# dmeoli/optiml

Measured on AMD Instinct MI355X. Metric: dual_qp_iterations_per_sec, higher is better.
Workload: dtype f64

## Files before the change

### optiml_amd/csrc/bq_api.hip

```cpp
#include <algorithm>
#include <chrono>
#include <cmath>
#include <cstdarg>
#include <cstdlib>

#include "bq_al.h"
#include "bq_c7.h"

static thread_local std::string g_last_error;

void bq_set_error(const char *fmt, ...) {
    char buf[1024];
    va_list ap;
    va_start(ap, fmt);
    vsnprintf(buf, sizeof(buf), fmt, ap);
    va_end(ap);
    g_last_error = buf;
}

extern "C" const char *bq_last_error(void) { return g_last_error.c_str(); }
extern "C" int bq_abi_version(void) { return BQ_ABI_VERSION; }

extern "C" int bq_device_count(int *count) {
    BQ_ARG(count != nullptr, "count is NULL");
// ... 692 lines not shown

extern "C" int bq_problem_eval(bq_problem *p, const double *x, double *f, double *g) {
    BQ_ARG(p && x && f, "NULL argument");
    BQ_HIP(hipSetDevice(p->ctx->device));
    BQ_TRY(upload_padded(p, x, p->va, p->N, p->ldN));
    BQ_TRY(bq_problem_apply(p, p->va, p->vb, nullptr));
    BQ_TRY(bq_vec_eval_f(p, p->va, p->vb, g ? p->vb : nullptr, p->scal));
    BQ_HIP(hipMemcpyAsync(f, p->scal, sizeof(double), hipMemcpyDeviceToHost, p->ctx->stream));
    if (g) BQ_HIP(hipMemcpyAsync(g, p->vb, sizeof(double) * p->N, hipMemcpyDeviceToHost, p->ctx->stream));
    BQ_SYNC(p->ctx);
    return BQ_OK;
}

extern "C" int bq_problem_gram_matvec(bq_problem *p, const double *w, double *out) {
    BQ_ARG(p && w && out, "NULL argument");
    BQ_ARG(p->kernel >= 0, "not a kernel-structured problem");
    bq_ctx *c = p->ctx;
    BQ_HIP(hipSetDevice(c->device));
    BQ_HIP(hipMemsetAsync(p->w, 0, sizeof(double) * p->ld, c->stream));
    BQ_HIP(hipMemcpyAsync(p->w, w, sizeof(double) * p->n, hipMemcpyHostToDevice, c->stream));
    BQ_TRY(bq_panel_product(p, false, p->w, nullptr));
    BQ_HIP(hipMemcpyAsync(out, p->s, sizeof(double) * p->n, hipMemcpyDeviceToHost, c->stream));
    BQ_SYNC(c);
    return BQ_OK;
}

extern "C" int bq_problem_panel_rows(bq_problem *p, int64_t row0, int64_t nrows, double *out) {
    BQ_ARG(p && out, "NULL argument");
    BQ_ARG(row0 >= p->r0 && row0 + nrows <= p->r1 && nrows >= 0, "rows outside this rank's block");
    BQ_ARG(!p->streamed, "a streamed problem keeps no panel");
    bq_ctx *c = p->ctx;
    BQ_HIP(hipSetDevice(c->device));
    if (nrows == 0) return BQ_OK;
    if (p->symmetric && p->compact) {
        const bq_c7p pv = bq_c7_view(p->panel, p->panel_elems);
        std::vector<uint32_t> lo((size_t)p->n);
        std::vector<uint16_t> mid((size_t)p->n);
        std::vector<uint8_t> top((size_t)p->n);
        for (int64_t r = 0; r < nrows; ++r) {
            const int64_t i = row0 + r;
            const int64_t len = std::min(p->n, bq_sym_pitch(i / BQ_SYM_TILE)), a = bq_sym_addr(i, 0, p->I0);
            BQ_HIP(hipMemcpyAsync(lo.data(), pv.lo + a, (size_t)len * 4, hipMemcpyDeviceToHost, c->stream));
            BQ_HIP(hipMemcpyAsync(mid.data(), pv.mid + a, (size_t)len * 2, hipMemcpyDeviceToHost, c->stream));
            BQ_HIP(hipMemcpyAsync(top.data(), pv.top + a, (size_t)len, hipMemcpyDeviceToHost, c->stream));
            BQ_SYNC(c);
            double *o = out + r * p->n;
            for (int64_t j = 0; j < len; ++j) {
                const uint64_t b = bq_c7_bits(lo[j], mid[j], top[j]);
                std::memcpy(&o[j], &b, sizeof(double));
            }
            for (int64_t j = len; j < p->n; ++j) o[j] = 0.0;
        }
        return BQ_OK;
    }
    if (p->symmetric) {
        const size_t esz = p->storage == BQ_F64 ? 8 : 4;
        std::vector<unsigned char> tmp((size_t)p->n * esz);
        for (int64_t r = 0; r < nrows; ++r) {
            const int64_t i = row0 + r;
            const int64_t len = std::min(p->n, bq_sym_pitch(i / BQ_SYM_TILE));
            BQ_HIP(hipMemcpyAsync(tmp.data(), (const unsigned char *)p->panel + (size_t)bq_sym_addr(i, 0, p->I0) * esz,
                                  (size_t)len * esz, hipMemcpyDeviceToHost, c->stream));
            BQ_SYNC(c);
            double *o = out + r * p->n;
            for (int64_t j = 0; j < len; ++j)
                o[j] = p->storage == BQ_F64 ? ((const double *)tmp.data())[j] : (double)((const float *)tmp.data())[j];
            for (int64_t j = len; j < p->n; ++j) o[j] = 0.0;
        }
        return BQ_OK;
    }
    const int64_t lr = row0 - p->r0;
    if (p->storage == BQ_F64) {
        BQ_HIP(hipMemcpy2DAsync(out, p->n * 8, (const double *)p->panel + lr * p->ld, p->ld * 8, p->n * 8, nrows,
                                hipMemcpyDeviceToHost, c->stream));
        BQ_SYNC(c);
    } else {
        std::vector<float> tmp((size_t)nrows * p->n);
        BQ_HIP(hipMemcpy2DAsync(tmp.data(), p->n * 4, (const float *)p->panel + lr * p->ld, p->ld * 4, p->n * 4, nrows,
                                hipMemcpyDeviceToHost, c->stream));
        BQ_SYNC(c);
        for (size_t i = 0; i < tmp.size(); ++i) out[i] = (double)tmp[i];
    }
    return BQ_OK;
}

extern "C" int bq_problem_time_matvec(bq_problem *p, int reps, double *mean_ms) {
    BQ_ARG(p && mean_ms && reps > 0, "argument");
    bq_ctx *c = p->ctx;
    BQ_HIP(hipSetDevice(c->device));
    hipEvent_t e0, e1;
    BQ_HIP(hipEventCreate(&e0));
    BQ_HIP(hipEventCreate(&e1));
    const bool prof = c->profiling;
    c->profiling = false;
    bq_seg_table tab;
    if (p->symmetric) bq_sym_seg_table(p, &tab);
    auto local = [&]() {
        if (p->streamed)
            return bq_stream_sym_product(c, p->stream_img, p->n, p->nb, tab, p->kernel, p->gamma, p->coef0, p->degree, p->add_one, p->w,
                                         p->s, 0, nullptr);
// ... 782 lines not shown
```

### optiml_amd/csrc/bq_common.h

```cpp
#pragma once
#include <hip/hip_runtime.h>

#include <atomic>
#include <cstdint>
#include <cstdio>
#include <cstring>
#include <string>
#include <vector>

#include "../../include/bcqp.h"

void bq_set_error(const char *fmt, ...);

#define BQ_HIP(expr)                                                                          \
    do {                                                                                      \
        hipError_t _e = (expr);                                                               \
        if (_e != hipSuccess) {                                                               \
            bq_set_error("%s failed at %s:%d: %s", #expr, __FILE__, __LINE__, hipGetErrorString(_e)); \
            return BQ_ERR_HIP;                                                                \
        }                                                                                     \
    } while (0)

#define BQ_TRY(expr)              \
    do {                          \
// ... 177 lines not shown
        int have = 0;
        std::vector<double> g, lp, lm;
        std::vector<unsigned char> mL, mU;
    };
    resume_t *resume = nullptr;
};

int bq_prof_begin(bq_ctx *ctx, int which, hipEvent_t *e0, hipEvent_t *e1, bool bracket = true);
int bq_prof_end(bq_ctx *ctx, int which, hipEvent_t e0, hipEvent_t e1, bool recorded = false);
void bq_prof_drop(bq_ctx *ctx, hipEvent_t e0, hipEvent_t e1);
void bq_prof_skip_arg(bq_ctx *ctx, hipEvent_t e0, int **slot, int *seq);
int bq_exchange_rows(bq_ctx *ctx, double *s, int64_t n, int64_t blk, int64_t r0, int64_t r1);
int bq_exchange_sum(bq_ctx *ctx, double *v, int64_t count);
int bq_exchange_gather(bq_ctx *ctx, double *buf, int64_t chunk);
void bq_problem_unref(bq_problem *p);
void bq_ctx_register(bq_ctx *c, bool alive);
void bq_ctx_drop_cache(bq_ctx *ctx);
void *bq_ctx_cache_take(bq_ctx *ctx, size_t bytes, size_t *cap);
void bq_ctx_cache_put(bq_ctx *ctx, void *panel, size_t bytes);
void bq_ctx_hold(bq_ctx *ctx, void *ptr, size_t bytes, const void *owner);
void bq_ctx_release_held(bq_ctx *ctx, const void *owner);

constexpr int BQ_F64C = 16;
struct bq_panel_ref {
    const void *base;
    int storage;
    int64_t elems;
};
static inline bq_panel_ref bq_problem_panel(const bq_problem *p, const void *base = nullptr) {
    return {base ? base : p->panel, p->compact ? BQ_F64C : p->storage, p->panel_elems};
}
static inline bool bq_compact_allowed() { return bq_hook_on("compact_panel"); }

constexpr int64_t BQ_SYM_TILE = 256;
__host__ __device__ inline int64_t bq_sym_off(int64_t I) { return BQ_SYM_TILE * BQ_SYM_TILE * (I * (I + 1) / 2); }
__host__ __device__ inline int64_t bq_sym_pitch(int64_t I) { return (I + 1) * BQ_SYM_TILE; }
__host__ __device__ inline int64_t bq_sym_addr(int64_t i, int64_t j, int64_t I0) {
    const int64_t I = i / BQ_SYM_TILE;
    return bq_sym_off(I) - bq_sym_off(I0) + (i - I * BQ_SYM_TILE) * bq_sym_pitch(I) + j;
}
constexpr int BQ_SYM_SEG = 8;
constexpr int BQ_SYM_SEG_MAX = 64;
static inline int bq_sym_segments(int world) { return BQ_SYM_SEG * ((world + BQ_SYM_SEG - 1) / BQ_SYM_SEG); }
int64_t bq_sym_seg_cut(int64_t nb, int s, int S);
static inline int bq_sym_seg_first(int rank, int world, int S) { return (int)((int64_t)rank * S / world); }
struct bq_seg_table {
    int count;
    int lo, hi;
    int slot[BQ_SYM_SEG_MAX];
    long long cut[BQ_SYM_SEG_MAX + 1];
};
struct bq_epilogue;
int bq_launch_symv(bq_ctx *ctx, const bq_panel_ref &panel, bool add_one, int64_t nb, const bq_seg_table &tab,
                   const double *w, double *slab, double *out, const int *done, const bq_epilogue *epi = nullptr);
int bq_launch_symv_segments(bq_ctx *ctx, const bq_panel_ref &panel, bool add_one, int64_t nb, const bq_seg_table &tab,
                            const double *w, double *slab, double *gath, const int *done);
int bq_launch_symv_segsum(bq_ctx *ctx, int64_t nb, const bq_seg_table &tab, const double *gath, double *out, const int *done,
                          const bq_epilogue *epi = nullptr);
void bq_sym_seg_table(const bq_problem *p, bq_seg_table *tab);
int bq_panel_product(bq_problem *p, bool add_one, const double *w, const int *done, const bq_epilogue *epi = nullptr,
                     bool *fused = nullptr);
constexpr int BQ_SYMM_CK = 4;
int64_t bq_symm_slab_len(int64_t nb);
int bq_launch_symm(bq_problem *p, bool add_one, const double *W, int64_t ldw, int slots, double *slab, double *out,
                   const int *nlive);
constexpr int BQ_SYMMW_CK = 16;
int64_t bq_symmw_slab_len(int64_t nb);
int bq_launch_symmw(bq_problem *p, bool add_one, const double *W, int64_t ldw, int slots, double *slab, double *out,
                    const int *nlive);
struct bq_pairs_plan;
int bq_pairs_plan_create(bq_problem *p, int ncls, const int *cls_tiles, int m, const int *pairs, bq_pairs_plan **out);
void bq_pairs_plan_destroy(bq_pairs_plan *pl);
int64_t bq_pairs_slab_len(const bq_pairs_plan *pl);
// ... 55 lines not shown
```

### optiml_amd/csrc/bq_dense.hip

```cpp
#include <algorithm>

#include "bq_common.h"

namespace {

template <typename T> struct bits_of;
template <> struct bits_of<double> {
    static __device__ __forceinline__ long long get(double v) { return __double_as_longlong(v); }
};
template <> struct bits_of<float> {
    static __device__ __forceinline__ long long get(float v) { return (long long)__float_as_int(v); }
};

template <typename T>
__global__ __launch_bounds__(256) void dense_pack_kernel(const double *__restrict__ tmp, int64_t ldt, int64_t width,
                                                         T *__restrict__ dst, int64_t pitch) {
    const int64_t r = blockIdx.y;
    for (int64_t c = (int64_t)blockIdx.x * 256 + threadIdx.x; c < width; c += (int64_t)gridDim.x * 256)
        dst[r * pitch + c] = (T)tmp[r * ldt + c];
}

template <typename T>
__global__ __launch_bounds__(256) void dense_mirror_diag_kernel(T *__restrict__ diag, int64_t pitch, int rows) {
    const int r = blockIdx.x, c = threadIdx.x;
    if (r < rows && c < rows && c > r) diag[(int64_t)r * pitch + c] = diag[(int64_t)c * pitch + r];
}

template <typename T>
__global__ __launch_bounds__(256) void dense_symcheck_kernel(const double *__restrict__ tmp, int64_t ldt, int64_t c_org, int64_t I,
                                                             int rows, int64_t c_lo, int64_t c_hi, const T *__restrict__ panel,
                                                             int64_t I0, int *__restrict__ flag) {
    __shared__ T tile[32][33];
    const int tx = threadIdx.x & 31, ty = threadIdx.x >> 5;
    const int64_t cb = c_lo + (int64_t)blockIdx.x * 32;
    const int rb = (int)blockIdx.y * 32;
    for (int k = ty; k < 32; k += 8) {
        const int64_t c = cb + k;
        const int r = rb + tx;
        T v = (T)0;
        if (c < c_hi && r < rows) v = panel[bq_sym_addr(c, I * BQ_SYM_TILE + r, I0)];
        tile[k][tx] = v;
    }
    __syncthreads();
    bool bad = false;
    for (int k = ty; k < 32; k += 8) {
        const int r = rb + k;
        const int64_t c = cb + tx;
        if (r < rows && c < c_hi) {
            const T mine = (T)tmp[(int64_t)r * ldt + (c - c_org)];
            bad = bad || bits_of<T>::get(mine) != bits_of<T>::get(tile[tx][k]);
        }
    }
// ... 4 lines not shown
int upload_sym_t(bq_problem *p, const double *Q, bool check, int *symmetric) {
    bq_ctx *c = p->ctx;
    const int64_t n = p->n, T256 = BQ_SYM_TILE;
    *symmetric = 1;
    if (p->I1 <= p->I0) return BQ_OK;
    struct scratch {
        double *tmp = nullptr;
        int *flag = nullptr;
        ~scratch() {
            if (tmp) hipFree(tmp);
            if (flag) hipFree(flag);
        }
    } s;
    const int64_t ldt = p->ld;
    BQ_HIP(hipMalloc(&s.tmp, sizeof(double) * (size_t)T256 * (size_t)ldt));
    BQ_HIP(hipMalloc(&s.flag, sizeof(int)));
    BQ_HIP(hipMemsetAsync(s.flag, 0, sizeof(int), c->stream));
    T *panel = reinterpret_cast<T *>(p->panel);
    const int64_t col_end = std::min(n, p->I1 * T256);
    int seen = 0, blocks = 0;
    auto look = [&]() -> int {
        BQ_HIP(hipMemcpyAsync(&seen, s.flag, sizeof(int), hipMemcpyDeviceToHost, c->stream));
        BQ_SYNC(c);
        return BQ_OK;
    };
    for (int64_t I = p->I1 - 1; I >= p->I0; --I) {
        const int rows = (int)std::min<int64_t>(T256, n - I * T256);
        if (rows <= 0) continue;
        const int64_t lower = std::min(n, (I + 1) * T256);
        const int64_t width = check ? col_end : lower;
        BQ_HIP(hipMemcpy2DAsync(s.tmp, (size_t)ldt * 8, Q + I * T256 * n, (size_t)n * 8, (size_t)width * 8, (size_t)rows,
                                hipMemcpyHostToDevice, c->stream));
        dense_pack_kernel<T><<<dim3((unsigned)std::min<int64_t>((lower + 255) / 256, 1024), (unsigned)rows), 256, 0, c->stream>>>(
            s.tmp, ldt, lower, panel + (bq_sym_off(I) - bq_sym_off(p->I0)), bq_sym_pitch(I));
        if (!check)
            dense_mirror_diag_kernel<T><<<(unsigned)rows, 256, 0, c->stream>>>(panel + (bq_sym_off(I) - bq_sym_off(p->I0)) + I * T256,
                                                                                bq_sym_pitch(I), rows);
        if (check) {
            const int64_t c_lo = I * T256;
            dense_symcheck_kernel<T><<<dim3((unsigned)((col_end - c_lo + 31) / 32), (unsigned)((rows + 31) / 32)), 256, 0, c->stream>>>(
                s.tmp, ldt, 0, I, rows, c_lo, col_end, panel, p->I0, s.flag);
            if (blocks == 0 || blocks % 32 == 31) {
                BQ_TRY(look());
                if (seen) break;
            }
        }
        ++blocks;
        BQ_HIP(hipGetLastError());
    }
    if (check && !seen && p->I0 > 0) {
        const int64_t c_lo = p->I0 * T256;
        for (int64_t Ib = 0; Ib < p->I0; ++Ib) {
            BQ_HIP(hipMemcpy2DAsync(s.tmp, (size_t)ldt * 8, Q + Ib * T256 * n + c_lo, (size_t)n * 8, (size_t)(col_end - c_lo) * 8,
                                    (size_t)T256, hipMemcpyHostToDevice, c->stream));
            dense_symcheck_kernel<T><<<dim3((unsigned)((col_end - c_lo + 31) / 32), (unsigned)(T256 / 32)), 256, 0, c->stream>>>(
                s.tmp, ldt, c_lo, Ib, (int)T256, c_lo, col_end, panel, p->I0, s.flag);
            if (Ib % 32 == 31) {
                BQ_TRY(look());
                if (seen) break;
            }
        }
        BQ_HIP(hipGetLastError());
    }
    if (check) {
        BQ_TRY(look());
        *symmetric = seen ? 0 : 1;
    }
    return BQ_OK;
}

// ... 75 lines not shown
```

### optiml_amd/csrc/bq_gram.hip

```cpp
#include "bq_c7.h"
#include "bq_common.h"

#include "bq_mfma_tile.h"
#include "bq_gram_image.h"

#include <type_traits>
#include <vector>

constexpr int GT = BQ_GT;
#ifndef BQ_STREAM_FOLD
#define BQ_STREAM_FOLD 0
#endif

template <typename T> struct gram_out {
    typedef T *__restrict__ ptr;
    typedef T *row;
};
template <> struct gram_out<bq_c7> {
    typedef bq_c7w ptr;
    typedef bq_c7w row;
};
template <typename T> __device__ __forceinline__ void store_elem(T *p, double v);
template <> __device__ __forceinline__ void store_elem<double>(double *p, double v) { __builtin_nontemporal_store(v, p); }
template <> __device__ __forceinline__ void store_elem<float>(float *p, double v) { __builtin_nontemporal_store((float)v, p); }
__device__ __forceinline__ void store_pair(double *p, double a, double b) {
    bq_d2 v;
    v.x = a;
    v.y = b;
    __builtin_nontemporal_store(v, reinterpret_cast<bq_d2 *>(p));
}
__device__ __forceinline__ void store_pair(float *p, double a, double b) {
    typedef float f2 __attribute__((ext_vector_type(2)));
    f2 v;
    v.x = (float)a;
    v.y = (float)b;
    __builtin_nontemporal_store(v, reinterpret_cast<f2 *>(p));
}

__device__ __forceinline__ void c7_flag(const bq_c7w &p, uint64_t a, uint64_t b) {
    if (!bq_c7_encodable(a) || !bq_c7_encodable(b)) *p.bad = 1;
}
__device__ __forceinline__ void store_pair(const bq_c7w &p, double a, double b) {
// ... 37 lines not shown
__global__ __launch_bounds__(256, 2) void gram_mfma_kernel(gram_params P, typename gram_out<T>::ptr out) {
    __shared__ __attribute__((aligned(16))) bq_tile_smem sm;
    int64_t bx = blockIdx.x, by = blockIdx.y;
    if (P.rect_rb > 0) {
        const int64_t b = blockIdx.x;
        const int64_t xcd = b & 7, slot = b >> 3;
        const int64_t rect = (slot / (GRAM_RECT_R * GRAM_RECT_S)) * 8 + xcd, idx = slot % (GRAM_RECT_R * GRAM_RECT_S);
        if (rect >= (int64_t)P.rect_rb * P.rect_sb) return;
        bx = (rect % P.rect_rb) * GRAM_RECT_R + idx % GRAM_RECT_R;
        by = (rect / P.rect_rb) * GRAM_RECT_S + idx / GRAM_RECT_R;
        if (bx >= P.tiles_m || by >= P.strips) return;
    }
    const int64_t arow = P.arow0 + bx * GT;
    int64_t tiles_n = (P.n + GT - 1) / GT;
    if (P.lower_only) {
        const int64_t lim = ((arow / BQ_SYM_TILE) + 1) * (BQ_SYM_TILE / GT);
        tiles_n = lim < tiles_n ? lim : tiles_n;
    }
    const int64_t j0 = by * GRAM_STRIP;
    const int64_t j1 = j0 + GRAM_STRIP < tiles_n ? j0 + GRAM_STRIP : tiles_n;
    if (j0 >= j1) return;
    const int lane = threadIdx.x & 63, wv = threadIdx.x >> 6;
    const int wr = wv >> 1, wc = wv & 1, ccol = lane & 15, crow = lane >> 4;
    const int64_t I0 = P.arow0 / BQ_SYM_TILE;
    __shared__ double rowsq[4][64];
    rowsq[wv][lane] = P.a2[arow + wr * 64 + lane];
    for (int64_t J = j0; J < j1; ++J) {
        const int64_t bcol = J * GT;
        bq_d4 acc[4][4];
        bq_tile_zero(acc);
        bq_mfma_tile_128(P.At, P.mp, arow, P.Bt, P.np, bcol, P.dp, sm, acc);
        int64_t opaque = 0;
        asm volatile("" : "+s"(opaque));
        const int64_t pitch = P.lower_only ? bq_sym_pitch(arow / BQ_SYM_TILE) : P.ld;
        const int64_t tile0 = P.lower_only ? bq_sym_addr(arow, 0, I0) : (arow - P.arow0) * P.ld;
        const typename gram_out<T>::row lane_base = out + tile0 + (int64_t)(wr * 64 + 2 * crow) * pitch + bcol + wc * 64 + 2 * ccol;
        double bj[4];
#pragma unroll
        for (int j = 0; j < 4; ++j) bj[j] = KIND == BQ_KERNEL_RBF ? P.b2[bcol + bq_acc_col(2 * (j >> 1)) + (j & 1)] : 0.0;
        auto epilogue = [&](auto on_diag, auto on_edge, auto deg) {
#pragma unroll
            for (int i = 0; i < 4; ++i) {
#pragma unroll
                for (int v = 0; v < 4; ++v) {
                    const int64_t gi = opaque + arow + bq_acc_row(i, v);
                    if (decltype(on_edge)::value && gi >= P.arow1) continue;
                    const auto rowp = lane_base + (opaque + (i >> 1) * 32 + 8 * v + (i & 1)) * pitch;
                    const double ai = rowsq[wv][bq_acc_row64(i, v)];
#pragma unroll
                    for (int jp = 0; jp < 2; ++jp) {
                        const int64_t gj = bcol + bq_acc_col(2 * jp);
                        if (decltype(on_edge)::value && gj >= P.n) continue;
                        double kv[2];
#pragma unroll
                        for (int h = 0; h < 2; ++h) {
                            const double dot = acc[i][2 * jp + h][v];
                            if (KIND == BQ_KERNEL_RBF) {
                                double dist = -2.0 * dot;
                                dist += ai;
                                dist += bj[2 * jp + h];
                                dist = fmax(dist, 0.0);
                                if (decltype(on_diag)::value && P.same && gi == gj + h) dist = 0.0;
                                kv[h] = bq_exp(-P.gamma * dist);
                            } else if (KIND == BQ_KERNEL_POLY) {
                                kv[h] = bq_poly_map<decltype(deg)::value>(P.gamma * dot + P.coef0, P.degree);
                            } else if (KIND == BQ_KERNEL_SIGMOID) {
                                kv[h] = tanh(P.gamma * dot + P.coef0);
                            } else {
                                kv[h] = dot;
// ... 599 lines not shown
```

### optiml_amd/csrc/bq_symm.hip

```cpp
#include "bq_common.h"
#include "bq_symv_tile.h"

constexpr int SJG = 2;
constexpr int SSR = 2;
static_assert(BQ_SYMM_CK * SSR == 8, "the row partials of a step are the eight values of the halving butterfly");

template <typename T, bool ADD_ONE>
__global__ __launch_bounds__(256, 2) void symm_tiles_kernel(bq_pptr<T> panel, int64_t nb, const double *__restrict__ W,
                                                          int64_t ldw, double *__restrict__ slab, const int *__restrict__ nlive, int ch) {
    constexpr int CK = BQ_SYMM_CK;
    if (ch * CK >= *nlive) return;
    __shared__ double colred[4][ST];
    const int64_t t = (int64_t)blockIdx.x;
    int64_t I = (int64_t)sqrt(2.0 * (double)SJG * (double)t);
    if (I >= nb) I = nb - 1;
    while (I > 0 && strips_before<SJG>(I) > t) --I;
    while (strips_before<SJG>(I + 1) <= t) ++I;
    const int64_t J0 = (t - strips_before<SJG>(I)) * SJG;
    const int nj = (int)((J0 + SJG <= I + 1) ? SJG : (I + 1 - J0));

    const int tid = threadIdx.x, lane = tid & 63, wv = tid >> 6;
    const int64_t pitch = bq_sym_pitch(I);
    const auto rows = panel + bq_sym_off(I) + (int64_t)(wv * 64) * pitch + J0 * ST;
    const double *Wc = W + (int64_t)ch * CK * ldw;
    const int c0 = tile_ld<T>::c0(lane), c1 = tile_ld<T>::c1(lane);
    d2_t wj0[CK][SJG], wj1[CK][SJG];
    double ca[CK][SJG][4];
#pragma unroll
    for (int c = 0; c < CK; ++c) {
#pragma unroll
        for (int j = 0; j < SJG; ++j) {
            const double *wJ = Wc + c * ldw + (J0 + (j < nj ? j : 0)) * ST;
            wj0[c][j] = *reinterpret_cast<const d2_t *>(wJ + c0);
            wj1[c][j] = *reinterpret_cast<const d2_t *>(wJ + c1);
            ca[c][j][0] = ca[c][j][1] = ca[c][j][2] = ca[c][j][3] = 0.0;
        }
    }
    const int64_t cs = nb * nb * ST;
    double *rowout = slab + (I * nb + J0) * ST + wv * 64;
    const bool b5 = lane & 32, b4 = lane & 16, b3 = lane & 8;

#pragma unroll 1
    for (int step = 0; step < 64 / SSR; ++step) {
        d2_t a[SJG][SSR], b[SJG][SSR];
#pragma unroll
        for (int j = 0; j < SJG; ++j) {
#pragma unroll
            for (int k = 0; k < SSR; ++k) {
                if (j < nj) {
                    tile_ld<T>::get(rows + (int64_t)(step * SSR + k) * pitch + j * ST, lane, a[j][k], b[j][k]);
                } else {
                    a[j][k] = (d2_t){0.0, 0.0};
                    b[j][k] = (d2_t){0.0, 0.0};
                }
            }
        }
// ... 105 lines not shown
```

### optiml_amd/csrc/bq_symmp.hip

```cpp
#include <algorithm>
#include <type_traits>
#include <vector>

#include "bq_common.h"
#include "bq_symv_tile.h"
#include "bq_symmw_step.h"
using namespace bq_mfma;

namespace {

constexpr int JG = 8;

struct pitem {
    int I, J0, nj, id;
};
struct pinfo {
    long long base;
    int L, na, ns;
    int a0, b0;
};

}

struct bq_pairs_plan {
// ... 28 lines not shown
    for (int p = 0; p < m; ++p) {
        const int a = pairs[2 * p], b = pairs[2 * p + 1];
        for (int I = ct[b]; I < ct[b + 1]; ++I)
            for (int J0 = ct[a]; J0 < ct[a + 1]; J0 += JG) single.push_back(pitem{I, J0, std::min(JG, ct[a + 1] - J0), p});
    }
    for (int c = 0; c < ncls; ++c) {
        if (cnt[c] == 0) continue;
        for (int I = ct[c]; I < ct[c + 1]; ++I)
            for (int J0 = ct[c]; J0 <= I; J0 += WJG) diag.push_back(pitem{I, J0, std::min(WJG, I + 1 - J0), c});
    }
}

static int64_t slab_len(const int *ct, int m, const int *pairs) {
    int64_t len = 0;
    for (int p = 0; p < m; ++p) {
        const int64_t L = (ct[pairs[2 * p] + 1] - ct[pairs[2 * p]]) + (ct[pairs[2 * p + 1] + 1] - ct[pairs[2 * p + 1]]);
        len += L * L * ST;
    }
    return len;
}


template <typename T, bool ADD_ONE, int SR>
__global__ __launch_bounds__(256, 2) void symmp_single_kernel(bq_pptr<T> panel, const pitem *__restrict__ items,
                                                              const pinfo *__restrict__ info, const int *__restrict__ plive,
                                                              const double *__restrict__ W, int64_t ldw, double *__restrict__ slab) {
    const pitem it = items[blockIdx.x];
    if (!plive[it.id]) return;
    __shared__ double colred[4][ST];
    const pinfo pi = info[it.id];
    const int64_t I = it.I, J0 = it.J0;
    const int nj = it.nj;
    const int tid = threadIdx.x, lane = tid & 63, wv = tid >> 6;
    const int64_t pitch = bq_sym_pitch(I);
    const auto rows = panel + bq_sym_off(I) + (int64_t)(wv * 64) * pitch + J0 * ST;
    const double *w = W + (int64_t)it.id * ldw;
    const double *wI = w + I * ST + wv * 64;
    const int c0 = tile_ld<T>::c0(lane), c1 = tile_ld<T>::c1(lane);
    d2_t wj0[JG], wj1[JG];
    double ca[JG][4];
#pragma unroll
    for (int j = 0; j < JG; ++j) {
        const double *wJ = w + (J0 + (j < nj ? j : 0)) * ST;
        wj0[j] = *reinterpret_cast<const d2_t *>(wJ + c0);
        wj1[j] = *reinterpret_cast<const d2_t *>(wJ + c1);
        ca[j][0] = ca[j][1] = ca[j][2] = ca[j][3] = 0.0;
    }
    const int64_t Il = pi.na + (I - pi.b0), Jl0 = J0 - pi.a0;
    double *ps = slab + pi.base;
    double *rowout = ps + (Il * pi.L + Jl0 / JG) * ST + wv * 64;
    const bool b5 = lane & 32, b4 = lane & 16;

#pragma unroll 1
    for (int step = 0; step < 64 / SR; ++step) {
        double rp[SR];
        double wi[SR];
#pragma unroll
        for (int k = 0; k < SR; ++k) {
            rp[k] = 0.0;
            wi[k] = wI[step * SR + k];
        }
#pragma unroll
        for (int j = 0; j < JG; ++j) {
            if (j < nj) {
                d2_t a[SR], b[SR];
#pragma unroll
                for (int k = 0; k < SR; ++k) {
                    const auto row = rows + (int64_t)(step * SR + k) * pitch + j * ST;
                    tile_ld<T>::get(row, lane, a[k], b[k]);
                }
#pragma unroll
                for (int k = 0; k < SR; ++k) {
                    if (ADD_ONE) {
                        a[k].x += 1.0;
                        a[k].y += 1.0;
                        b[k].x += 1.0;
                        b[k].y += 1.0;
                    }
                    rp[k] = fma(b[k].y, wj1[j].y, fma(b[k].x, wj1[j].x, fma(a[k].y, wj0[j].y, fma(a[k].x, wj0[j].x, rp[k]))));
                    ca[j][0] = fma(a[k].x, wi[k], ca[j][0]);
                    ca[j][1] = fma(a[k].y, wi[k], ca[j][1]);
                    ca[j][2] = fma(b[k].x, wi[k], ca[j][2]);
                    ca[j][3] = fma(b[k].y, wi[k], ca[j][3]);
                }
            }
        }
        double s1;
        int rho;
        if constexpr (SR == 8) {
            const bool b3 = lane & 8;
            double u[4], t2[2];
#pragma unroll
            for (int i = 0; i < 4; ++i) {
                const double send = b5 ? rp[i] : rp[i + 4];
                const double keep = b5 ? rp[i + 4] : rp[i];
                u[i] = keep + __shfl_xor(send, 32, 64);
            }
#pragma unroll
            for (int i = 0; i < 2; ++i) {
                const double send = b4 ? u[i] : u[i + 2];
                const double keep = b4 ? u[i + 2] : u[i];
// ... 43 lines not shown

template <typename T, bool ADD_ONE>
__global__ __launch_bounds__(256, 2) void symmp_diag_kernel(bq_pptr<T> panel, const pitem *__restrict__ items,
                                                            const pinfo *__restrict__ info, const int *__restrict__ pairs,
                                                            const int *__restrict__ ct, const int *__restrict__ ccnt,
                                                            const int *__restrict__ cslot, int kpad, const double *__restrict__ W,
                                                            int64_t ldw, double *__restrict__ slab) {
    const pitem it = items[blockIdx.x];
    const int cls = it.id, ch = blockIdx.y;
    const int live = ccnt[cls] - ch * CK;
    if (live <= 0) return;
    __shared__ double tb[4][16 * TP];
    __shared__ double wj[ST * WP];
    __shared__ long long sbase[CK];
    __shared__ int sL[CK], soff[CK], shoff[CK], spair[CK];
    const int tid = threadIdx.x, lane = tid & 63, wv = tid >> 6, h = lane >> 4, s = lane & 15;
    const int64_t I = it.I, J0 = it.J0, C0 = ct[cls];
    const int nj = it.nj;
    if (tid < CK) {
        int q = -1;
        if (tid < live) {
            q = cslot[cls * kpad + ch * CK + tid];
            const pinfo pi = info[q];
            const bool first = pairs[2 * q] == cls;
            sbase[tid] = pi.base;
            sL[tid] = pi.L;
            soff[tid] = first ? 0 : pi.na;
            shoff[tid] = first ? 0 : pi.ns;
        }
        spair[tid] = q;
    }
    __syncthreads();

    const int64_t pitch = bq_sym_pitch(I);
    const auto base = panel + bq_sym_off(I) + (int64_t)(wv * 64 + s) * pitch + J0 * ST;
    auto rowp = [&](int j, int cq, int st) { return base + (int64_t)(16 * st) * pitch + j * ST + 64 * cq; };

    const int myq = spair[s];
    double wi[4][4];
#pragma unroll
    for (int st = 0; st < 4; ++st)
#pragma unroll
        for (int u = 0; u < 4; ++u) wi[st][u] = myq >= 0 ? W[(int64_t)myq * ldw + I * ST + wv * 64 + 16 * st + 4 * u + h] : 0.0;
    d4_t acc1[4];
#pragma unroll
    for (int st = 0; st < 4; ++st) acc1[st] = (d4_t){0.0, 0.0, 0.0, 0.0};
    double *img = tb[wv];

    typename step_ld<T>::raw cur, nxt;
    step_ld<T>::load(rowp(0, 0, 0), h, cur);
    const int nquart = nj * 4;
#pragma unroll 1
    for (int qk = 0; qk < nquart; ++qk) {
        const int j = qk >> 2, cq = qk & 3;
        const bool diag = J0 + j == I;
        if (cq == 0) {
            __syncthreads();
            const int64_t r = (J0 + j) * ST + tid;
#pragma unroll
            for (int c = 0; c < CK; ++c) wj[tid * WP + c] = spair[c] >= 0 ? W[(int64_t)spair[c] * ldw + r] : 0.0;
            __syncthreads();
        }
        d4_t acc2[4];
#pragma unroll
        for (int jc = 0; jc < 4; ++jc) acc2[jc] = (d4_t){0.0, 0.0, 0.0, 0.0};
#pragma unroll
        for (int st = 0; st < 4; ++st) {
            if (st < 3) step_ld<T>::load(rowp(j, cq, st + 1), h, nxt);
            else if (qk + 1 < nquart) step_ld<T>::load(rowp((qk + 1) >> 2, (qk + 1) & 3, 0), h, nxt);
// ... 256 lines not shown
```

### optiml_amd/csrc/bq_symmw.hip

```cpp
#include "bq_common.h"
#include "bq_symv_tile.h"
#include "bq_symmw_step.h"
using namespace bq_mfma;

template <typename T, bool ADD_ONE>
__global__ __launch_bounds__(256, 2) void symmw_tiles_kernel(bq_pptr<T> panel, int64_t nb, const double *__restrict__ W,
                                                          int64_t ldw, double *__restrict__ slab, const int *__restrict__ nlive, int ch) {
    const int live = *nlive - ch * CK;
    if (live <= 0) return;
    __shared__ double tb[4][16 * TP];
    __shared__ double wj[ST * WP];
    const int64_t sidx = (int64_t)blockIdx.x;
    int64_t I = (int64_t)sqrt(2.0 * (double)WJG * (double)sidx);
    if (I >= nb) I = nb - 1;
    while (I > 0 && strips_before<WJG>(I) > sidx) --I;
    while (strips_before<WJG>(I + 1) <= sidx) ++I;
    const int64_t J0 = (sidx - strips_before<WJG>(I)) * WJG;
    const int nj = (int)((J0 + WJG <= I + 1) ? WJG : (I + 1 - J0));

    const int tid = threadIdx.x, lane = tid & 63, wv = tid >> 6, h = lane >> 4, s = lane & 15;
    const int64_t pitch = bq_sym_pitch(I);
    const double *Wc = W + (int64_t)ch * CK * ldw;
    const int64_t cs = nb * nb * ST;
    const auto base = panel + bq_sym_off(I) + (int64_t)(wv * 64 + s) * pitch + J0 * ST;
    auto rowp = [&](int j, int cq, int st) { return base + (int64_t)(16 * st) * pitch + j * ST + 64 * cq; };

    double wi[4][4];
#pragma unroll
    for (int st = 0; st < 4; ++st)
#pragma unroll
        for (int u = 0; u < 4; ++u) wi[st][u] = Wc[s * ldw + I * ST + wv * 64 + 16 * st + 4 * u + h];
    d4_t acc1[4];
#pragma unroll
    for (int st = 0; st < 4; ++st) acc1[st] = (d4_t){0.0, 0.0, 0.0, 0.0};
    double *img = tb[wv];

    typename step_ld<T>::raw cur, nxt;
    step_ld<T>::load(rowp(0, 0, 0), h, cur);
    const int nquart = nj * 4;
#pragma unroll 1
    for (int qk = 0; qk < nquart; ++qk) {
        const int j = qk >> 2, cq = qk & 3;
        const bool diag = J0 + j == I;
        if (cq == 0) {
            __syncthreads();
            const double *wJ = Wc + (J0 + j) * ST + tid;
#pragma unroll
            for (int c = 0; c < CK; ++c) wj[tid * WP + c] = wJ[c * ldw];
            __syncthreads();
        }
        d4_t acc2[4];
#pragma unroll
        for (int jc = 0; jc < 4; ++jc) acc2[jc] = (d4_t){0.0, 0.0, 0.0, 0.0};
#pragma unroll
        for (int st = 0; st < 4; ++st) {
            if (st < 3) step_ld<T>::load(rowp(j, cq, st + 1), h, nxt);
            else if (qk + 1 < nquart) step_ld<T>::load(rowp((qk + 1) >> 2, (qk + 1) & 3, 0), h, nxt);
// ... 77 lines not shown
```

### optiml_amd/csrc/bq_symv.hip

```cpp
#include <cstdlib>

#include <hip/hip_ext.h>

#include "bq_common.h"
#include "bq_epilogue.h"
#include "bq_symv_tile.h"

constexpr int JG_DEFAULT = 8;

template <typename T, bool ADD_ONE, int JG, int SR>
__global__ __launch_bounds__(256, 2) void symv_tiles_kernel(bq_pptr<T> panel, int64_t I0, int64_t nb,
                                                          const double *__restrict__ w, double *__restrict__ slab,
                                                          const int *__restrict__ done, int *__restrict__ skip, int skip_seq) {
    if (done != nullptr && *done) {
        if (skip != nullptr && blockIdx.x == 0 && threadIdx.x == 0) *skip = skip_seq;
        return;
    }
    __shared__ double colred[4][ST];
    const int64_t t = (int64_t)blockIdx.x + strips_before<JG>(I0);
    int64_t I = (int64_t)sqrt(2.0 * (double)JG * (double)t);
    if (I >= nb) I = nb - 1;
    while (I > 0 && strips_before<JG>(I) > t) --I;
    while (strips_before<JG>(I + 1) <= t) ++I;
    const int64_t g = t - strips_before<JG>(I);
    const int64_t J0 = g * JG;
    const int nj = (int)((J0 + JG <= I + 1) ? JG : (I + 1 - J0));

    const int tid = threadIdx.x, lane = tid & 63, wv = tid >> 6;
    const int64_t pitch = bq_sym_pitch(I);
    const auto rows = panel + (bq_sym_off(I) - bq_sym_off(I0)) + (int64_t)(wv * 64) * pitch + J0 * ST;
    const double *wI = w + I * ST + wv * 64;
    const int c0 = tile_ld<T>::c0(lane), c1 = tile_ld<T>::c1(lane);
    d2_t wj0[JG], wj1[JG];
    double ca[JG][4];
#pragma unroll
    for (int j = 0; j < JG; ++j) {
        const double *wJ = w + (J0 + (j < nj ? j : 0)) * ST;
        wj0[j] = *reinterpret_cast<const d2_t *>(wJ + c0);
        wj1[j] = *reinterpret_cast<const d2_t *>(wJ + c1);
        ca[j][0] = ca[j][1] = ca[j][2] = ca[j][3] = 0.0;
    }
    double *rowout = slab + (I * nb + J0) * ST + wv * 64;
    const bool b5 = lane & 32, b4 = lane & 16;

#pragma unroll 1
    for (int step = 0; step < 64 / SR; ++step) {
        double rp[SR];
        double wi[SR];
#pragma unroll
        for (int k = 0; k < SR; ++k) {
            rp[k] = 0.0;
            wi[k] = wI[step * SR + k];
        }
#pragma unroll
        for (int j = 0; j < JG; ++j) {
            if (j < nj) {
                d2_t a[SR], b[SR];
#pragma unroll
                for (int k = 0; k < SR; ++k) {
                    const auto row = rows + (int64_t)(step * SR + k) * pitch + j * ST;
                    tile_ld<T>::get(row, lane, a[k], b[k]);
                }
#pragma unroll
// ... 242 lines not shown
```

Baseline: 183.4.

## Pack symmetric panel rows in strips of eight column tiles

Changes the packed lower-triangular panel layout so each row block is stored as strips of 2048 columns with a short pitch, instead of one full-width row. The symv, symm, symmw, symmp, Gram and dense-pack kernels now compute addresses per strip, so a kernel block's rows sit close together and pitch strides stay small, which should improve memory locality in the iteration matvec. Host-side row extraction is rewritten as batched 2D copies per strip. Addressing now costs more arithmetic, and symmp must handle a group that spans two strips.

```diff
diff --git a/optiml_amd/csrc/bq_api.hip b/optiml_amd/csrc/bq_api.hip
--- a/optiml_amd/csrc/bq_api.hip
+++ b/optiml_amd/csrc/bq_api.hip
@@ -748,40 +748,49 @@
     bq_ctx *c = p->ctx;
     BQ_HIP(hipSetDevice(c->device));
     if (nrows == 0) return BQ_OK;
-    if (p->symmetric && p->compact) {
-        const bq_c7p pv = bq_c7_view(p->panel, p->panel_elems);
-        std::vector<uint32_t> lo((size_t)p->n);
-        std::vector<uint16_t> mid((size_t)p->n);
-        std::vector<uint8_t> top((size_t)p->n);
-        for (int64_t r = 0; r < nrows; ++r) {
-            const int64_t i = row0 + r;
-            const int64_t len = std::min(p->n, bq_sym_pitch(i / BQ_SYM_TILE)), a = bq_sym_addr(i, 0, p->I0);
-            BQ_HIP(hipMemcpyAsync(lo.data(), pv.lo + a, (size_t)len * 4, hipMemcpyDeviceToHost, c->stream));
-            BQ_HIP(hipMemcpyAsync(mid.data(), pv.mid + a, (size_t)len * 2, hipMemcpyDeviceToHost, c->stream));
-            BQ_HIP(hipMemcpyAsync(top.data(), pv.top + a, (size_t)len, hipMemcpyDeviceToHost, c->stream));
+    if (p->symmetric) {
+        const int64_t n = p->n;
+        const size_t esz = p->compact ? 4 : p->storage == BQ_F64 ? 8 : 4;
+        const int64_t cap = std::min<int64_t>(nrows, BQ_SYM_TILE);
+        std::vector<unsigned char> lo((size_t)cap * n * esz);
+        std::vector<uint16_t> mid(p->compact ? (size_t)cap * n : 0);
+        std::vector<uint8_t> top(p->compact ? (size_t)cap * n : 0);
+        const bq_c7p pv = p->compact ? bq_c7_view(p->panel, p->panel_elems) : bq_c7p{nullptr, nullptr, nullptr};
+        for (int64_t r = 0; r < nrows;) {
+            const int64_t i0 = row0 + r, I = i0 / BQ_SYM_TILE;
+            const int64_t rb = std::min(nrows - r, (I + 1) * BQ_SYM_TILE - i0);
+            const int64_t len = std::min(n, bq_sym_cols(I));
+            for (int64_t j0 = 0; j0 < len; j0 += BQ_SYM_STRIP_COLS) {
+                const int64_t a = bq_sym_addr(i0, j0, p->I0), m = std::min(len - j0, BQ_SYM_STRIP_COLS);
+                const int64_t w = bq_sym_strip_w(I, j0 / BQ_SYM_STRIP_COLS);
+                const unsigned char *src = p->compact ? (const unsigned char *)(pv.lo + a) : (const unsigned char *)p->panel + (size_t)a * esz;
+                BQ_HIP(hipMemcpy2DAsync(lo.data() + (size_t)j0 * esz, (size_t)n * esz, src, (size_t)w * esz, (size_t)m * esz, (size_t)rb,
+                                        hipMemcpyDeviceToHost, c->stream));
+                if (p->compact) {
+                    BQ_HIP(hipMemcpy2DAsync(mid.data() + j0, (size_t)n * 2, pv.mid + a, (size_t)w * 2, (size_t)m * 2, (size_t)rb,
+                                            hipMemcpyDeviceToHost, c->stream));
+                    BQ_HIP(hipMemcpy2DAsync(top.data() + j0, (size_t)n, pv.top + a, (size_t)w, (size_t)m, (size_t)rb,
+                                            hipMemcpyDeviceToHost, c->stream));
+                }
+            }
             BQ_SYNC(c);
-            double *o = out + r * p->n;
-            for (int64_t j = 0; j < len; ++j) {
-                const uint64_t b = bq_c7_bits(lo[j], mid[j], top[j]);
-                std::memcpy(&o[j], &b, sizeof(double));
+            for (int64_t k = 0; k < rb; ++k) {
+                double *o = out + (r + k) * n;
+                if (p->compact) {
+                    const uint32_t *l = (const uint32_t *)lo.data() + k * n;
+                    for (int64_t j = 0; j < len; ++j) {
+                        const uint64_t b = bq_c7_bits(l[j], mid[(size_t)(k * n + j)], top[(size_t)(k * n + j)]);
+                        std::memcpy(&o[j], &b, sizeof(double));
+                    }
+                } else if (p->storage == BQ_F64) {
+                    std::memcpy(o, (const double *)lo.data() + k * n, (size_t)len * 8);
+                } else {
+                    const float *f = (const float *)lo.data() + k * n;
+                    for (int64_t j = 0; j < len; ++j) o[j] = (double)f[j];
+                }
+                for (int64_t j = len; j < n; ++j) o[j] = 0.0;
             }
-            for (int64_t j = len; j < p->n; ++j) o[j] = 0.0;
-        }
-        return BQ_OK;
-    }
-    if (p->symmetric) {
-        const size_t esz = p->storage == BQ_F64 ? 8 : 4;
-        std::vector<unsigned char> tmp((size_t)p->n * esz);
-        for (int64_t r = 0; r < nrows; ++r) {
-            const int64_t i = row0 + r;
-            const int64_t len = std::min(p->n, bq_sym_pitch(i / BQ_SYM_TILE));
-            BQ_HIP(hipMemcpyAsync(tmp.data(), (const unsigned char *)p->panel + (size_t)bq_sym_addr(i, 0, p->I0) * esz,
-                                  (size_t)len * esz, hipMemcpyDeviceToHost, c->stream));
-            BQ_SYNC(c);
-            double *o = out + r * p->n;
-            for (int64_t j = 0; j < len; ++j)
-                o[j] = p->storage == BQ_F64 ? ((const double *)tmp.data())[j] : (double)((const float *)tmp.data())[j];
-            for (int64_t j = len; j < p->n; ++j) o[j] = 0.0;
+            r += rb;
         }
         return BQ_OK;
     }
diff --git a/optiml_amd/csrc/bq_common.h b/optiml_amd/csrc/bq_common.h
--- a/optiml_amd/csrc/bq_common.h
+++ b/optiml_amd/csrc/bq_common.h
@@ -233,13 +233,7 @@
 }
 static inline bool bq_compact_allowed() { return bq_hook_on("compact_panel"); }
 
-constexpr int64_t BQ_SYM_TILE = 256;
-__host__ __device__ inline int64_t bq_sym_off(int64_t I) { return BQ_SYM_TILE * BQ_SYM_TILE * (I * (I + 1) / 2); }
-__host__ __device__ inline int64_t bq_sym_pitch(int64_t I) { return (I + 1) * BQ_SYM_TILE; }
-__host__ __device__ inline int64_t bq_sym_addr(int64_t i, int64_t j, int64_t I0) {
-    const int64_t I = i / BQ_SYM_TILE;
-    return bq_sym_off(I) - bq_sym_off(I0) + (i - I * BQ_SYM_TILE) * bq_sym_pitch(I) + j;
-}
+#include "bq_sym_layout.h"
 constexpr int BQ_SYM_SEG = 8;
 constexpr int BQ_SYM_SEG_MAX = 64;
 static inline int bq_sym_segments(int world) { return BQ_SYM_SEG * ((world + BQ_SYM_SEG - 1) / BQ_SYM_SEG); }
diff --git a/optiml_amd/csrc/bq_dense.hip b/optiml_amd/csrc/bq_dense.hip
--- a/optiml_amd/csrc/bq_dense.hip
+++ b/optiml_amd/csrc/bq_dense.hip
@@ -14,10 +14,10 @@
 
 template <typename T>
 __global__ __launch_bounds__(256) void dense_pack_kernel(const double *__restrict__ tmp, int64_t ldt, int64_t width,
-                                                         T *__restrict__ dst, int64_t pitch) {
+                                                         T *__restrict__ panel, int64_t I, int64_t I0) {
     const int64_t r = blockIdx.y;
     for (int64_t c = (int64_t)blockIdx.x * 256 + threadIdx.x; c < width; c += (int64_t)gridDim.x * 256)
-        dst[r * pitch + c] = (T)tmp[r * ldt + c];
+        panel[bq_sym_addr(I * BQ_SYM_TILE + r, c, I0)] = (T)tmp[r * ldt + c];
 }
 
 template <typename T>
@@ -88,10 +88,10 @@
         BQ_HIP(hipMemcpy2DAsync(s.tmp, (size_t)ldt * 8, Q + I * T256 * n, (size_t)n * 8, (size_t)width * 8, (size_t)rows,
                                 hipMemcpyHostToDevice, c->stream));
         dense_pack_kernel<T><<<dim3((unsigned)std::min<int64_t>((lower + 255) / 256, 1024), (unsigned)rows), 256, 0, c->stream>>>(
-            s.tmp, ldt, lower, panel + (bq_sym_off(I) - bq_sym_off(p->I0)), bq_sym_pitch(I));
+            s.tmp, ldt, lower, panel, I, p->I0);
         if (!check)
-            dense_mirror_diag_kernel<T><<<(unsigned)rows, 256, 0, c->stream>>>(panel + (bq_sym_off(I) - bq_sym_off(p->I0)) + I * T256,
-                                                                                bq_sym_pitch(I), rows);
+            dense_mirror_diag_kernel<T><<<(unsigned)rows, 256, 0, c->stream>>>(panel + bq_sym_addr(I * T256, I * T256, p->I0),
+                                                                                bq_sym_strip_w(I, I / BQ_SYM_STRIP), rows);
         if (check) {
             const int64_t c_lo = I * T256;
             dense_symcheck_kernel<T><<<dim3((unsigned)((col_end - c_lo + 31) / 32), (unsigned)((rows + 31) / 32)), 256, 0, c->stream>>>(
diff --git a/optiml_amd/csrc/bq_gram.hip b/optiml_amd/csrc/bq_gram.hip
--- a/optiml_amd/csrc/bq_gram.hip
+++ b/optiml_amd/csrc/bq_gram.hip
@@ -8,6 +8,7 @@
 #include <vector>
 
 constexpr int GT = BQ_GT;
+static_assert(BQ_SYM_STRIP_COLS % GT == 0 && BQ_SYM_TILE % GT == 0, "a Gram tile lies inside one strip of the packed layout");
 #ifndef BQ_STREAM_FOLD
 #define BQ_STREAM_FOLD 0
 #endif
@@ -111,9 +112,9 @@
         bq_mfma_tile_128(P.At, P.mp, arow, P.Bt, P.np, bcol, P.dp, sm, acc);
         int64_t opaque = 0;
         asm volatile("" : "+s"(opaque));
-        const int64_t pitch = P.lower_only ? bq_sym_pitch(arow / BQ_SYM_TILE) : P.ld;
-        const int64_t tile0 = P.lower_only ? bq_sym_addr(arow, 0, I0) : (arow - P.arow0) * P.ld;
-        const typename gram_out<T>::row lane_base = out + tile0 + (int64_t)(wr * 64 + 2 * crow) * pitch + bcol + wc * 64 + 2 * ccol;
+        const int64_t pitch = P.lower_only ? bq_sym_strip_w(arow / BQ_SYM_TILE, bcol / BQ_SYM_STRIP_COLS) : P.ld;
+        const int64_t tile0 = P.lower_only ? bq_sym_addr(arow, bcol, I0) : (arow - P.arow0) * P.ld + bcol;
+        const typename gram_out<T>::row lane_base = out + tile0 + (int64_t)(wr * 64 + 2 * crow) * pitch + wc * 64 + 2 * ccol;
         double bj[4];
 #pragma unroll
         for (int j = 0; j < 4; ++j) bj[j] = KIND == BQ_KERNEL_RBF ? P.b2[bcol + bq_acc_col(2 * (j >> 1)) + (j & 1)] : 0.0;
diff --git a/optiml_amd/csrc/bq_sym_layout.h b/optiml_amd/csrc/bq_sym_layout.h
--- /dev/null
+++ b/optiml_amd/csrc/bq_sym_layout.h
@@ -0,0 +1,25 @@
+#pragma once
+#include <cstdint>
+
+#if defined(__HIPCC__)
+#define BQ_HD __host__ __device__
+#else
+#define BQ_HD
+#endif
+
+constexpr int64_t BQ_SYM_TILE = 256;
+constexpr int64_t BQ_SYM_STRIP = 8;
+constexpr int64_t BQ_SYM_STRIP_COLS = BQ_SYM_STRIP * BQ_SYM_TILE;
+BQ_HD inline int64_t bq_sym_off(int64_t I) { return BQ_SYM_TILE * BQ_SYM_TILE * (I * (I + 1) / 2); }
+BQ_HD inline int64_t bq_sym_cols(int64_t I) { return (I + 1) * BQ_SYM_TILE; }
+BQ_HD inline int64_t bq_sym_strip_w(int64_t I, int64_t g) {
+    const int64_t rest = bq_sym_cols(I) - g * BQ_SYM_STRIP_COLS;
+    return rest < BQ_SYM_STRIP_COLS ? rest : BQ_SYM_STRIP_COLS;
+}
+BQ_HD inline int64_t bq_sym_strip_off(int64_t I, int64_t g) {
+    return bq_sym_off(I) + g * (BQ_SYM_TILE * BQ_SYM_STRIP_COLS);
+}
+BQ_HD inline int64_t bq_sym_addr(int64_t i, int64_t j, int64_t I0) {
+    const int64_t I = i / BQ_SYM_TILE, g = j / BQ_SYM_STRIP_COLS;
+    return bq_sym_strip_off(I, g) - bq_sym_off(I0) + (i - I * BQ_SYM_TILE) * bq_sym_strip_w(I, g) + (j - g * BQ_SYM_STRIP_COLS);
+}
diff --git a/optiml_amd/csrc/bq_symm.hip b/optiml_amd/csrc/bq_symm.hip
--- a/optiml_amd/csrc/bq_symm.hip
+++ b/optiml_amd/csrc/bq_symm.hip
@@ -20,8 +20,9 @@
     const int nj = (int)((J0 + SJG <= I + 1) ? SJG : (I + 1 - J0));
 
     const int tid = threadIdx.x, lane = tid & 63, wv = tid >> 6;
-    const int64_t pitch = bq_sym_pitch(I);
-    const auto rows = panel + bq_sym_off(I) + (int64_t)(wv * 64) * pitch + J0 * ST;
+    static_assert(BQ_SYM_STRIP % SJG == 0, "a strip of this kernel lies inside one strip of the layout");
+    const int64_t gl = J0 / BQ_SYM_STRIP, pitch = bq_sym_strip_w(I, gl);
+    const auto rows = panel + (bq_sym_strip_off(I, gl) + (int64_t)(__builtin_amdgcn_readfirstlane(wv) * 64) * pitch + (J0 - gl * BQ_SYM_STRIP) * ST);
     const double *Wc = W + (int64_t)ch * CK * ldw;
     const int c0 = tile_ld<T>::c0(lane), c1 = tile_ld<T>::c1(lane);
     d2_t wj0[CK][SJG], wj1[CK][SJG];
diff --git a/optiml_amd/csrc/bq_symmp.hip b/optiml_amd/csrc/bq_symmp.hip
--- a/optiml_amd/csrc/bq_symmp.hip
+++ b/optiml_amd/csrc/bq_symmp.hip
@@ -84,16 +84,22 @@
     const int64_t I = it.I, J0 = it.J0;
     const int nj = it.nj;
     const int tid = threadIdx.x, lane = tid & 63, wv = tid >> 6;
-    const int64_t pitch = bq_sym_pitch(I);
-    const auto rows = panel + bq_sym_off(I) + (int64_t)(wv * 64) * pitch + J0 * ST;
     const double *w = W + (int64_t)it.id * ldw;
     const double *wI = w + I * ST + wv * 64;
     const int c0 = tile_ld<T>::c0(lane), c1 = tile_ld<T>::c1(lane);
     d2_t wj0[JG], wj1[JG];
     double ca[JG][4];
+    static_assert(JG <= BQ_SYM_STRIP, "a strip of this kernel straddles at most two strips of the layout");
+    const int64_t gA = J0 / BQ_SYM_STRIP;
+    const int jsplit = (int)((gA + 1) * BQ_SYM_STRIP - J0);
+    const int64_t pA = bq_sym_strip_w(I, gA), pB = bq_sym_strip_w(I, gA + 1);
+    const int64_t wrow = (int64_t)(__builtin_amdgcn_readfirstlane(wv) * 64);
+    const int64_t oA = bq_sym_strip_off(I, gA) + wrow * pA + (J0 - gA * BQ_SYM_STRIP) * ST;
+    const int64_t oB = bq_sym_strip_off(I, gA + 1) + wrow * pB - jsplit * ST;
 #pragma unroll
     for (int j = 0; j < JG; ++j) {
-        const double *wJ = w + (J0 + (j < nj ? j : 0)) * ST;
+        const int64_t J = J0 + (j < nj ? j : 0);
+        const double *wJ = w + J * ST;
         wj0[j] = *reinterpret_cast<const d2_t *>(wJ + c0);
         wj1[j] = *reinterpret_cast<const d2_t *>(wJ + c1);
         ca[j][0] = ca[j][1] = ca[j][2] = ca[j][3] = 0.0;
@@ -112,13 +118,16 @@
             rp[k] = 0.0;
             wi[k] = wI[step * SR + k];
         }
+        int so = step * SR;
+        asm volatile("" : "+s"(so));
 #pragma unroll
         for (int j = 0; j < JG; ++j) {
             if (j < nj) {
                 d2_t a[SR], b[SR];
 #pragma unroll
                 for (int k = 0; k < SR; ++k) {
-                    const auto row = rows + (int64_t)(step * SR + k) * pitch + j * ST;
+                    const int64_t rel = (int64_t)(unsigned)((so + k) * (j < jsplit ? (int)pA : (int)pB) + j * ST);
+                    const auto row = panel + ((j < jsplit ? oA : oB) + rel);
                     tile_ld<T>::get(row, lane, a[k], b[k]);
                 }
 #pragma unroll
@@ -228,9 +237,10 @@
     }
     __syncthreads();
 
-    const int64_t pitch = bq_sym_pitch(I);
-    const auto base = panel + bq_sym_off(I) + (int64_t)(wv * 64 + s) * pitch + J0 * ST;
-    auto rowp = [&](int j, int cq, int st) { return base + (int64_t)(16 * st) * pitch + j * ST + 64 * cq; };
+    auto rowp = [&](int j, int cq, int st) {
+        const int64_t J = J0 + j, gl = J / BQ_SYM_STRIP, pitch = bq_sym_strip_w(I, gl);
+        return panel + (bq_sym_strip_off(I, gl) + (J - gl * BQ_SYM_STRIP) * ST + 64 * cq) + (int64_t)(wv * 64 + 16 * st + s) * pitch;
+    };
 
     const int myq = spair[s];
     double wi[4][4];
diff --git a/optiml_amd/csrc/bq_symmw.hip b/optiml_amd/csrc/bq_symmw.hip
--- a/optiml_amd/csrc/bq_symmw.hip
+++ b/optiml_amd/csrc/bq_symmw.hip
@@ -19,10 +19,11 @@
     const int nj = (int)((J0 + WJG <= I + 1) ? WJG : (I + 1 - J0));
 
     const int tid = threadIdx.x, lane = tid & 63, wv = tid >> 6, h = lane >> 4, s = lane & 15;
-    const int64_t pitch = bq_sym_pitch(I);
+    static_assert(BQ_SYM_STRIP % WJG == 0, "a strip of this kernel lies inside one strip of the layout");
+    const int64_t gl = J0 / BQ_SYM_STRIP, pitch = bq_sym_strip_w(I, gl);
     const double *Wc = W + (int64_t)ch * CK * ldw;
     const int64_t cs = nb * nb * ST;
-    const auto base = panel + bq_sym_off(I) + (int64_t)(wv * 64 + s) * pitch + J0 * ST;
+    const auto base = panel + bq_sym_strip_off(I, gl) + (int64_t)(wv * 64 + s) * pitch + (J0 - gl * BQ_SYM_STRIP) * ST;
     auto rowp = [&](int j, int cq, int st) { return base + (int64_t)(16 * st) * pitch + j * ST + 64 * cq; };
 
     double wi[4][4];
diff --git a/optiml_amd/csrc/bq_symv.hip b/optiml_amd/csrc/bq_symv.hip
--- a/optiml_amd/csrc/bq_symv.hip
+++ b/optiml_amd/csrc/bq_symv.hip
@@ -27,8 +27,9 @@
     const int nj = (int)((J0 + JG <= I + 1) ? JG : (I + 1 - J0));
 
     const int tid = threadIdx.x, lane = tid & 63, wv = tid >> 6;
-    const int64_t pitch = bq_sym_pitch(I);
-    const auto rows = panel + (bq_sym_off(I) - bq_sym_off(I0)) + (int64_t)(wv * 64) * pitch + J0 * ST;
+    static_assert(JG == BQ_SYM_STRIP, "the strip of the kernel is the strip of the layout");
+    const int64_t pitch = bq_sym_strip_w(I, g);
+    const auto rows = panel + ((bq_sym_strip_off(I, g) - bq_sym_off(I0)) + (int64_t)(__builtin_amdgcn_readfirstlane(wv) * 64) * pitch);
     const double *wI = w + I * ST + wv * 64;
     const int c0 = tile_ld<T>::c0(lane), c1 = tile_ld<T>::c1(lane);
     d2_t wj0[JG], wj1[JG];
```

Result: faster. 187.0 (median of 6 runs) (+2.0%).
